# lixiaobai09/xgnn

Hardware: AMD Instinct MI355X
Metric: sampled edges/s + feature-extract GB/s per epoch-step (higher is better)
Workload: dtype u32 ids / f32 rows (bit copy)

## Files before the change

xgnn_amd/csrc/engine/engine.cc:

```cpp
#include "engine.h"
#include "team.h"
#include "../labor_hash.h"
#include "../row_formats.h"

#include <fcntl.h>
#include <pthread.h>
#include <sys/mman.h>
#include <signal.h>
#include <sys/stat.h>
#include <sys/wait.h>
#include <unistd.h>

#include <algorithm>
#include <atomic>
#include <chrono>
#include <condition_variable>
#include <cstdio>
#include <cstdlib>
#include <cstring>
#include <fstream>
#include <iostream>
#include <memory>
#include <mutex>
#include <random>
// ... 130 lines not shown
      if (kv.count("queue_timeout_s")) cfg.queue_timeout_s = std::stod(kv["queue_timeout_s"]);
      if (!(cfg.queue_timeout_s > 0))
        fatal(__FILE__, __LINE__, "arch5: queue_timeout_s = " + kv["queue_timeout_s"] + ": a positive number of seconds");
      cfg.num_worker = cfg.num_sample_worker + cfg.num_train_worker;
      break;
    }
    case kArch6:
      SAM_CHECK(kv.count("num_worker"), "arch6 needs num_worker");
      cfg.num_worker = std::stoull(kv["num_worker"]);
      SAM_CHECK(cfg.num_worker >= 1, "num_worker >= 1");
      break;
    default:
      fatal(__FILE__, __LINE__, "only arch0 (CPU), arch1 (standalone), arch3 (dedicated), arch4 (dedicated with prefetch), "
                                "arch5 (factored) and arch6 (SGNN/XGNN) are built; see DESIGN.md");
  }
  if (cfg.sample_type != GGMS_RANDOM_WALK) {
    SAM_CHECK(kv.count("num_fanout") && kv.count("fanout"), "khop sampling needs num_fanout/fanout");
    size_t nf = std::stoull(kv["num_fanout"]);
    std::stringstream ss(kv["fanout"]);
    for (size_t i = 0; i < nf; ++i) {
      size_t f = 0;
      ss >> f;
      SAM_CHECK(f > 0, "fanout: num_fanout positive integers expected");
      cfg.fanout.push_back(f);
    }
  } else {
    cfg.random_walk_length = std::stoull(kv["random_walk_length"]);
    cfg.random_walk_restart_prob = std::stod(kv["random_walk_restart_prob"]);
    cfg.num_random_walk = std::stoull(kv["num_random_walk"]);
    cfg.num_neighbor = std::stoull(kv["num_neighbor"]);
    SAM_CHECK(cfg.random_walk_length > 0 && cfg.num_random_walk > 0 && cfg.num_neighbor > 0,
              "random walk needs random_walk_length, num_random_walk and num_neighbor >= 1");
    cfg.fanout.assign(cfg.num_layer, cfg.num_neighbor);
  }
  if (kv.count("use_dist_graph")) {
    cfg.dist_graph_percentage = std::stod(kv["use_dist_graph"]);
    cfg.use_dist_graph = cfg.dist_graph_percentage > 0.0;
  }
  if (kv.count("part_cache") && kv["part_cache"] == "True") {
    SAM_CHECK(cfg.arch == kArch6, "partition cache can only be used in arch6");
    cfg.part_cache = true;
  }
  if (kv.count("gpu_extract") && kv["gpu_extract"] == "True") cfg.gpu_extract = (cfg.arch == kArch6);
  if (kv.count("replicate_percentage")) cfg.replicate_percentage = std::stod(kv["replicate_percentage"]);
  if (kv.count("presample_epoch")) cfg.presample_epoch = std::stoull(kv["presample_epoch"]);
  if (kv.count("seed")) { cfg.has_seed = true; cfg.seed = std::stoull(kv["seed"]); }
  if (kv.count("hash_table")) cfg.direct_table = kv["hash_table"] != "hashed";
  if (kv.count("lookahead")) cfg.lookahead = std::stoull(kv["lookahead"]);
  if (kv.count("staged_serial_epochs")) cfg.staged_serial_epochs = std::stoull(kv["staged_serial_epochs"]);
  if (kv.count("staged_serial_steps")) cfg.staged_serial_steps = std::stoull(kv["staged_serial_steps"]);
  if (kv.count("extract_streams")) cfg.extract_streams = std::max<size_t>(1, std::min<size_t>(2, std::stoull(kv["extract_streams"])));
  if (const char *e = getenv("SAMGRAPH_EXTRACT_STREAMS")) cfg.extract_streams = (e[0] == '1') ? 1 : 2;
  if (kv.count("pipelines")) cfg.pipelines = std::max<size_t>(1, std::min<size_t>(4, std::stoull(kv["pipelines"])));
  if (cfg.lookahead + 1 < cfg.pipelines) cfg.pipelines = cfg.lookahead + 1;
  if (cfg.arch == kArch5) {
    cfg.lookahead = 0;
    cfg.pipelines = 1;
  }
  SAM_CHECK(cfg.sample_type >= GGMS_KHOP0 && cfg.sample_type <= GGMS_KHOP_LABOR, "unknown sample type");
  if (cfg.sample_type == GGMS_KHOP_LABOR && cfg.arch == kArch0)
    fatal(__FILE__, __LINE__, "arch0: _sample_type 8 (khop_labor) is not supported: the CPU engine has no sampler for "
                              "it; it samples with khop0 or khop2");
  cfg.labor_seed = cfg.has_seed ? cfg.seed : (uint64_t)std::chrono::system_clock::now().time_since_epoch().count();
  if (kv.count("feat_out_dtype")) {
    static const std::map<std::string, int> names = {{"f32", GGMS_F32}, {"f16", GGMS_F16}, {"bf16", GGMS_BF16}};
    const std::string v = kv["feat_out_dtype"];
    if (!names.count(v))
      fatal(__FILE__, __LINE__, "feat_out_dtype = " + v + ": the converting gather delivers f32, f16 or bf16");
    cfg.feat_out_dtype = names.at(v);
    if (cfg.arch == kArch0)
      fatal(__FILE__, __LINE__, "arch0: feat_out_dtype is not built for the CPU engine: its extractor copies rows, it does "
                                "not convert them");
    if (cfg.arch == kArch6 && !cfg.gpu_extract && cfg.cache_percentage < 1.0)
      fatal(__FILE__, __LINE__, "arch6: feat_out_dtype needs gpu_extract = True or cache_percentage 1.0: the host-staged "
                                "tier's rows land in the batch by hipMemcpyAsync, which does not convert");
  }
  if (kv.count("feat_store_dtype")) {
    const std::string v = kv["feat_store_dtype"];
    const auto name = kFeatDtypeNames.find(v);
    if (name == kFeatDtypeNames.end() || !ggms::quantiser_writes(name->second))
      fatal(__FILE__, __LINE__, "feat_store_dtype = " + v + ": unknown store type; the GPU quantiser writes F16, BF16, "
                                "F8E4M3, F8E5M2 or Q8ROW");
    cfg.feat_store_dtype = name->second;
    if (cfg.arch == kArch0)
      fatal(__FILE__, __LINE__, "arch0: feat_store_dtype needs a GPU: the table is encoded by a kernel, and the CPU engine "
                                "has no GPU; quantise the dataset offline (datagen.quantize_features)");
    if (cfg.arch == kArch5 || cfg.arch == kArch6)
      fatal(__FILE__, __LINE__, std::string(cfg.arch == kArch5 ? "arch5" : "arch6") + ": feat_store_dtype is not built: the "
                                "process that loads the dataset forks its workers and must not initialise the GPU before it "
                                "forks; quantise the dataset offline (datagen.quantize_features)");
    if (cfg.feat_store_dtype == GGMS_Q8ROW && cfg.feat_out_dtype < 0) fatal(__FILE__, __LINE__, kQ8RowNeedsOutDtype);
  }
  if (kv.count("task")) {
    const std::string v = kv["task"];
    if (v != "node_classification" && v != "link_prediction")
      fatal(__FILE__, __LINE__, "task = " + v + ": node_classification (the default) or link_prediction");
    cfg.link_prediction = v == "link_prediction";
  }
  if (cfg.link_prediction) {
    static const char *const arch_names[] = {"arch0", "arch1", "arch2", "arch3", "arch4", "arch5", "arch6", "arch7"};
    if (cfg.arch != kArch1)
      fatal(__FILE__, __LINE__, std::string(arch_names[cfg.arch]) + ": task = link_prediction is not built: edge seeds, "
                                "negative sampling and the pair ids run in arch1's sampling chain only");
    if (cfg.sample_type == GGMS_RANDOM_WALK)
      fatal(__FILE__, __LINE__, "task = link_prediction with _sample_type 3 (random_walk) is not built: the pair ids are "
                                "the k-hop batch's seed ids");
// ... 599 lines not shown
  const size_t isz = num_cache_node / P + (p < num_cache_node % P ? 1 : 0) + 1;
  std::vector<uint32_t> pip(isz);
  size_t ecount = 0;
  for (uint32_t v = p; v < num_cache_node; v += P) ecount += indptr[v + 1] - indptr[v];
  std::vector<uint32_t> pix(std::max<size_t>(ecount, 1));
  uint32_t cnt = 0;
  for (uint32_t v = p; v < num_cache_node; v += P) {
    const uint32_t ne = indptr[v + 1] - indptr[v];
    pip[v / P] = cnt;
    std::memcpy(&pix[cnt], &indices[indptr[v]], ne * 4ull);
    cnt += ne;
  }
  pip[isz - 1] = cnt;
  part_indptr_.assign(P + 1, nullptr);
  part_indices_.assign(P + 1, nullptr);
  part_indptr_[p] = dev_upload(pip.data(), isz * 4, stream_);
  part_indices_[p] = dev_upload(pix.data(), ecount * 4, stream_);
  SAM_HIP(hipStreamSynchronize(stream_));
  if (P > 1) {
    SAM_HIP(hipIpcGetMemHandle(&shared_->graph_indptr[p], part_indptr_[p]));
    SAM_HIP(hipIpcGetMemHandle(&shared_->graph_indices[p], part_indices_[p]));
    shared_->indptr_words[p] = isz;
    shared_->indices_words[p] = ecount;
    Barrier("graph shards published");
    for (uint32_t q = 0; q < P; ++q) {
      if (q == p) continue;
      part_indptr_[q] = OpenPeer(shared_->graph_indptr[q], q, shared_->indptr_words[q] * 4, "graph indptr shard");
      part_indices_[q] = OpenPeer(shared_->graph_indices[q], q, shared_->indices_words[q] * 4, "graph indices shard");
    }
    Barrier("graph shards opened");
  }
  part_indptr_[P] = dev_upload(ds.indptr.ptr, ds.indptr.bytes, stream_);
  SAM_HIP(hipStreamSynchronize(stream_));
  part_indices_[P] = (void *)map_host(ds.indices.ptr, ds.indices.bytes);
  SAM_CHECK(P <= GGMS_MAX_PARTS, "use_dist_graph: at most GGMS_MAX_PARTS topology shards");
  graph_.part_indptr = (const ggms_id_t *const *)part_indptr_.data();
  graph_.part_indices = (const ggms_id_t *const *)part_indices_.data();
  graph_.num_part = P;
  graph_.num_cache_node = num_cache_node;
}

void Engine::ComputeBounds() {
  const uint32_t L = (uint32_t)cfg.fanout.size();
  max_seeds_ = (size_t)(cfg.batch_size * 1.25) + 1;
  if (cfg.link_prediction) max_seeds_ = cfg.batch_size * (2 + cfg.num_negative);
  max_input_.resize(L);
  max_edges_.resize(L);
  SAM_GGMS(ggms_sample_batch_capacity(max_seeds_, cfg.fanout.data(), L, max_input_.data(), max_edges_.data(), &max_unique_));
  if (cfg.arch == kArch4)
    SAM_GGMS(ggms_sample_batch_prefetch_capacity(max_seeds_, cfg.fanout.data(), L, (const ggms_id_t *)ds.indptr.ptr,
                                                 ds.num_node, cfg.prefetch_max_edges, &max_prefetch_edges_, &max_unique_));
}

void Engine::SampleInit(int worker_id, const std::string &ctx) {
  SAM_CHECK(data_ready_, "samgraph_data_init first");
  if (cfg.arch == kArch5) {
    SAM_CHECK(role_ == kRoleNone, "arch5: a process is one sampler or one trainer (one sample_init or one train_init)");
    SAM_CHECK(worker_id >= 0 && (size_t)worker_id < cfg.num_sample_worker, "arch5: sample_init(worker_id) with 0 <= "
              "worker_id < num_sample_worker = " + std::to_string(cfg.num_sample_worker));
    role_ = kRoleSampler;
  }
  worker_id_ = worker_id;
  device_ = parse_device(ctx);
  trainer_device_ = Dedicated() ? cfg.trainer_device : device_;
  if (trainer_device_ != device_) EnablePeerAccess();
  SAM_HIP(hipSetDevice(device_));
  SAM_HIP(hipStreamCreateWithFlags(&stream_, hipStreamNonBlocking));
  if (cfg.arch != kArch5) {
    SAM_HIP(hipSetDevice(trainer_device_));
    SAM_HIP(hipStreamCreateWithFlags(&stream_extract_, hipStreamNonBlocking));
    if (cfg.extract_streams > 1) SAM_HIP(hipStreamCreateWithFlags(&stream_extract2_, hipStreamNonBlocking));
    SAM_HIP(hipSetDevice(device_));
  }
  UploadGraph();
  ShufflerInit();
  const uint32_t L = (uint32_t)cfg.fanout.size();
  ComputeBounds();
  std::memset(&ht_, 0, sizeof(ht_));
  ht_.direct = cfg.direct_table ? 1 : 0;
  ht_.o2n_size = cfg.direct_table ? ds.num_node : ggms_hashtable_num_buckets(max_unique_);
  ht_.n2o_size = max_unique_;
  SAM_HIP(hipMalloc(&ht_.o2n, ht_.o2n_size * (cfg.direct_table ? 8 : 16)));
  SAM_HIP(hipMalloc((void **)&ht_.n2o, max_unique_ * 4));
  SAM_HIP(hipMalloc((void **)&ht_.num_items_dev, 16));
  SAM_GGMS(ggms_hashtable_init(&ht_, stream_));
  std::memset(&extra_, 0, sizeof(extra_));
  if (cfg.sample_type == GGMS_WEIGHTED_KHOP || cfg.sample_type == GGMS_WEIGHTED_KHOP_HASH_DEDUP) {
    d_prob_ = dev_upload(ds.prob_table.ptr, ds.prob_table.bytes, stream_);
    d_alias_ = dev_upload(ds.alias_table.ptr, ds.alias_table.bytes, stream_);
    extra_.prob_table = (const float *)d_prob_;
    extra_.alias_table = (const ggms_id_t *)d_alias_;
  }
  if (cfg.sample_type == GGMS_WEIGHTED_KHOP_PREFIX) {
    d_prob_ = dev_upload(ds.prob_table.ptr, ds.prob_table.bytes, stream_);
    extra_.prob_table = (const float *)d_prob_;
  }
  extra_.random_walk_length = cfg.random_walk_length;
  extra_.random_walk_restart_prob = cfg.random_walk_restart_prob;
  extra_.num_random_walk = cfg.num_random_walk;
  if (cfg.sample_type == GGMS_KHOP_LABOR) {
    num_states_ = 0;
    states_ = nullptr;
  } else {
    num_states_ = ggms_random_states_count(cfg.sample_type, cfg.fanout.data(), L, max_seeds_, cfg.num_random_walk);
    size_t max_in = 0;
    for (auto v : max_input_) max_in = std::max(max_in, v);
    num_states_ = std::max(num_states_, (max_in + 127) / 128 * 8);
    num_states_ = std::max(num_states_, (max_in + 1023) / 1024 * 256);
    if (cfg.sample_type == GGMS_RANDOM_WALK)
      num_states_ = std::max(num_states_, ggms_random_walk_num_states(max_in, cfg.num_random_walk));
    SAM_HIP(hipMalloc(&states_, num_states_ * GGMS_RNG_STATE_BYTES));
    const uint64_t seed = cfg.has_seed ? cfg.seed + 1000003ull * worker_id
                                       : (uint64_t)std::chrono::system_clock::now().time_since_epoch().count();
    SAM_GGMS(ggms_random_states_init(states_, num_states_, seed, stream_));
  }
  ws_bytes_ = cfg.arch == kArch4 ? ggms_sample_batch_prefetch_workspace_bytes(cfg.sample_type, max_seeds_, cfg.fanout.data(),
                                                                          L, &extra_, max_prefetch_edges_)
                                 : ggms_sample_batch_workspace_bytes(cfg.sample_type, max_seeds_, cfg.fanout.data(), L, &extra_);
  SAM_HIP(hipMalloc(&ws_, ws_bytes_));
  pipes_.assign(cfg.pipelines, Pipe{});
  for (size_t p = 0; p < pipes_.size(); ++p) {
    Pipe &P = pipes_[p];
    SAM_HIP(hipEventCreateWithFlags(&P.rng_done, hipEventDisableTiming));
    if (p == 0) {
      P.stream = stream_;
      P.ht = ht_;
      P.ws = ws_;
      continue;
    }
    SAM_HIP(hipStreamCreateWithFlags(&P.stream, hipStreamNonBlocking));
    P.ht = ht_;
    SAM_HIP(hipMalloc(&P.ht.o2n, ht_.o2n_size * (cfg.direct_table ? 8 : 16)));
    SAM_HIP(hipMalloc((void **)&P.ht.n2o, max_unique_ * 4));
    SAM_HIP(hipMalloc((void **)&P.ht.num_items_dev, 16));
    SAM_GGMS(ggms_hashtable_init(&P.ht, stream_));
    SAM_HIP(hipMalloc(&P.ws, ws_bytes_));
  }
  if (cfg.link_prediction && cfg.exclude_seed_edges) {
    drop_ws_bytes_ = ggms_drop_pair_edges_workspace_bytes(cfg.batch_size, max_edges_.data(), L);
    SAM_CHECK(drop_ws_bytes_ > 0, "exclude_seed_edges: the batch bounds are out of ggms_drop_pair_edges' range");
    for (Pipe &P : pipes_) SAM_HIP(hipMalloc(&P.drop_ws, drop_ws_bytes_));
  }
  if (cfg.edge_ids) {
    eid_ws_bytes_ = ggms_edge_positions_workspace_bytes(max_edges_.data(), L);
    SAM_CHECK(eid_ws_bytes_ > 0, "edge_ids: the batch bounds are out of ggms_edge_positions' range");
    for (Pipe &P : pipes_) SAM_HIP(hipMalloc(&P.eid_ws, eid_ws_bytes_));
  }
  SAM_HIP(hipStreamSynchronize(stream_));
  prof.Resize(cfg.num_epoch, num_global_step_);
  if (cfg.UsePresample()) {
    auto t0 = std::chrono::steady_clock::now();
    if (worker_id_ == 0) Presample();
    if (cfg.arch == kArch5) {
      if (worker_id_ == 0) PublishRanking();
      else WaitRankingReady();
    } else {
      Barrier("presample ranking");
    }
    prof.LogInit( 8, std::chrono::duration<double>(std::chrono::steady_clock::now() - t0).count());
  }
  if (cfg.arch == kArch5) {
    sbatch_ = std::make_unique<Batch>();
    Batch *b = sbatch_.get();
    b->sampler.Alloc(max_edges_, max_unique_, max_seeds_, cfg.sample_type == GGMS_RANDOM_WALK);
    SAM_HIP(hipEventCreateWithFlags(&b->ev_sampled, hipEventDisableTiming));
    SAM_HIP(hipEventCreateWithFlags(&b->ev_done, hipEventDisableTiming));
    QueueMap();
  }
  sample_ready_ = true;
}

void Engine::EnablePeerAccess() {
  int can = 0;
  SAM_HIP(hipDeviceCanAccessPeer(&can, trainer_device_, device_));
  if (!can)
    fatal(__FILE__, __LINE__, "arch3: GPU " + std::to_string(trainer_device_) + " (trainer_ctx) cannot access GPU " +
                                  std::to_string(device_) + " (sampler_ctx) (hipDeviceCanAccessPeer): the trainer GPU "
                                  "reads each sampled batch from the sampler GPU's memory, which needs peer access");
  SAM_HIP(hipSetDevice(trainer_device_));
  const hipError_t e = hipDeviceEnablePeerAccess(device_, 0);
  if (e == hipErrorPeerAccessAlreadyEnabled) (void)hipGetLastError();
  else SAM_HIP(e);
  SAM_HIP(hipSetDevice(device_));
  log_info("arch3: peer access GPU " + std::to_string(trainer_device_) + " -> GPU " + std::to_string(device_) + " enabled");
}

void Engine::Presample() {
  const uint32_t L = (uint32_t)cfg.fanout.size();
  const size_t n_train = ds.num_train;
  const size_t steps = (n_train + cfg.batch_size - 1) / cfg.batch_size;
  const bool closure = cfg.cache_policy == 4 ;
  std::vector<uint32_t> data((const uint32_t *)ds.train_set.ptr, (const uint32_t *)ds.train_set.ptr + n_train);
  uint32_t *d_train = nullptr, *d_freq = nullptr;
  uint64_t *d_counts = nullptr;
  SAM_HIP(hipMalloc((void **)&d_train, std::max<size_t>(n_train, 1) * 4));
  SAM_HIP(hipMalloc((void **)&d_freq, ds.num_node * 4));
  SAM_HIP(hipMalloc((void **)&d_counts, CountsBytes(L)));
  SAM_HIP(hipMemsetAsync(d_freq, 0, ds.num_node * 4, stream_));
  uint32_t *d_visit = nullptr, *d_closure = nullptr;
  void *d_cws = nullptr;
// ... 287 lines not shown
    b->trainer.Alloc(max_edges_, max_unique_, max_seeds_, cfg.sample_type == GGMS_RANDOM_WALK);
    SAM_HIP(hipMalloc(&b->feat, max_unique_ * batch_feat_row_bytes()));
    SAM_HIP(hipMalloc((void **)&b->label, max_seeds_ * 8));
    if (cfg.link_prediction) {
      SAM_HIP(hipMalloc((void **)&b->edge_ids, cfg.batch_size * 4));
      SAM_HIP(hipMalloc((void **)&b->seed_ids, max_seeds_ * 4));
      if (cfg.exclude_seed_edges) {
        SAM_HIP(hipMalloc((void **)&b->excluded_dev, L * 8));
        SAM_HIP(hipHostMalloc((void **)&b->excluded, L * 8));
        std::memset(b->excluded, 0, L * 8);
      }
    }
    if (cfg.edge_ids) {
      b->eid.assign(L, nullptr);
      b->efeat.assign(L, nullptr);
      for (uint32_t i = 0; i < L; ++i) {
        SAM_HIP(hipMalloc((void **)&b->eid[i], std::max<size_t>(max_edges_[i], 4) * 4));
        if (cfg.edge_feat) SAM_HIP(hipMalloc(&b->efeat[i], std::max<size_t>(max_edges_[i] * ds.edge_feat_row_bytes(), 16)));
      }
    }
    if (StagedHostTier()) {
      if (cache_table_) {
        for (uint32_t **p : {&b->miss_src, &b->miss_dst, &b->hit_src, &b->hit_dst}) SAM_HIP(hipMalloc((void **)p, max_unique_ * 4));
        SAM_HIP(hipMalloc(&b->idx_ws, ggms_cache_index_workspace_bytes(max_unique_)));
        SAM_HIP(hipMalloc(&b->miss_rows_dev, max_unique_ * row_bytes));
      }
      SAM_HIP(hipEventCreateWithFlags(&b->ev_ids, hipEventDisableTiming));
      SAM_HIP(hipHostMalloc(&b->miss_rows_host, max_unique_ * row_bytes));
      SAM_HIP(hipHostMalloc((void **)&b->miss_ids_host, max_unique_ * 4));
    }
    SAM_HIP(hipHostMalloc((void **)&b->counts, CountsBytes(L)));
    std::memset(b->counts, 0, CountsBytes(L));
    SAM_HIP(hipEventCreateWithFlags(&b->ev_seeds, hipEventDisableTiming));
    SAM_HIP(hipEventCreateWithFlags(&b->ev_label, hipEventDisableTiming));
    SAM_HIP(hipEventCreate(&b->ev_xstart));
    SAM_HIP(hipEventCreate(&b->ev_done));
    SAM_GGMS(ggms_launch_timer_create(&b->gather_timer));
    if (BatchSampledElsewhere()) SAM_GGMS(ggms_launch_timer_create(&b->handoff_timer));
    if (Dedicated()) {
      SAM_HIP(hipSetDevice(device_));
      b->sampler.Alloc(max_edges_, max_unique_, max_seeds_, cfg.sample_type == GGMS_RANDOM_WALK);
    } else {
      b->sampler = b->trainer;
    }
    SAM_HIP(hipEventCreate(&b->ev_start));
    SAM_HIP(hipEventCreate(&b->ev_sampled));
    if (cfg.arch == kArch4) {
      SAM_HIP(hipEventCreate(&b->ev_expand));
      SAM_HIP(hipEventCreate(&b->ev_final));
    }
    SAM_HIP(hipSetDevice(trainer_device_));
    slots_.push_back(std::move(b));
  }
  train_ready_ = true;
}

void Engine::Init() {
  if (cfg.arch == kArch0) {
    CpuInit();
    return;
  }
  DataInit();
  const std::string ctx = "cuda:" + std::to_string(cfg.sampler_device);
  SampleInit(0, ctx);
  TrainInit(0, "cuda:" + std::to_string(cfg.trainer_device));
}

void Engine::Start() {
  if (Dedicated()) ExtractStart(0);
}

void Engine::Shutdown() {
  shutdown_ = true;
  bg_stop_ = true;
  pool_cv_.notify_all();
  if (bg_.joinable()) bg_.join();
  if (cfg.arch == kArch0) CpuShutdown();
  for (auto &P : pipes_)
    if (P.stream) (void)hipStreamSynchronize(P.stream);
  if (stream_) (void)hipStreamSynchronize(stream_);
  if (stream_extract_) (void)hipStreamSynchronize(stream_extract_);
  if (stream_extract2_) (void)hipStreamSynchronize(stream_extract2_);
}

Batch *Engine::AcquireSlot(bool background) {
  for (;;) {
    {
      std::lock_guard<std::mutex> lk(pool_mu_);
      for (auto &b : slots_)
        if (!b->in_use && b->refs.load() == 0) { b->in_use = true; return b.get(); }
    }
    if (bg_stop_) return nullptr;
    if (!background) return nullptr;
    std::this_thread::sleep_for(std::chrono::microseconds(20));
  }
}

void Engine::RunSampleOnce(bool background) {
  if (IsArch5Sampler()) {
    SendOne();
    return;
  }
  if (background) {
    (void)EnqueueOne(true);
    return;
  }
  ++fg_calls_;
  while (fg_enqueued_ < fg_calls_ + cfg.lookahead && EnqueueOne(false)) ++fg_enqueued_;
}

bool Engine::EnqueueOne(bool background) {
  if (cfg.arch == kArch0) return CpuEnqueueOne(background);
  SAM_CHECK(train_ready_, "engine not initialised");
  struct RestoreDevice {
    int dev = -1;
    ~RestoreDevice() { if (dev >= 0) (void)hipSetDevice(dev); }
  } restore;
  if (Dedicated()) SAM_HIP(hipGetDevice(&restore.dev));
  SAM_HIP(hipSetDevice(device_));
  Batch *b = AcquireSlot(background);
  if (!b) return false;
  if (cfg.arch == kArch5) {
    if (!Receive(b)) {
      std::lock_guard<std::mutex> lk(pool_mu_);
      b->in_use = false;
      return false;
    }
    ++enq_count_;
    EnqueueGather(b, nullptr);
    return true;
  }
  Pipe &P = pipes_[enq_count_ % pipes_.size()];
  hipStream_t ss = P.stream;
  if (!ShufflerNext(b, ss)) {
    std::lock_guard<std::mutex> lk(pool_mu_);
    b->in_use = false;
    return false;
  }
  ++enq_count_;
  SAM_HIP(hipEventRecord(b->ev_start, ss));
  SampleInto(b, P);
  EnqueueGather(b, ss);
  return true;
}

void Engine::SampleInto(Batch *b, Pipe &P) {
  const uint32_t L = (uint32_t)cfg.fanout.size();
  const BatchArrays &s = b->sampler;
  ggms_sample_extra_t extra = extra_;
  extra.data = s.data.data();
  extra.seeds_distinct = BatchSeedsDistinct(cur_step_ * cfg.batch_size, b->num_seeds) ? 1u : 0u;
  extra.labor_salt = ggms::labor_batch_salt(cfg.labor_seed, b->key / num_global_step_, b->key % num_global_step_);
  if (cfg.link_prediction) {
    uint64_t *forced = s.counts_dev + GGMS_COUNT_LINK_FORCED(L);
    SAM_HIP(hipMemsetAsync(forced, 0, 8, P.stream));
    const uint32_t salt = ggms::fmix32(extra.labor_salt ^ 0x6c696e6bu);
    SAM_GGMS(ggms_link_seeds(&graph_, b->edge_ids, b->num_pos, cfg.num_negative, cfg.negative_mode, salt, s.output_nodes,
                             forced, P.stream));
    extra.seeds_distinct = 0;
  }
  if (pipes_.size() > 1 && cfg.sample_type != GGMS_KHOP0 && cfg.sample_type != GGMS_KHOP_LABOR) {
    extra.rng_wait = last_rng_done_;
    extra.rng_done = P.rng_done;
    last_rng_done_ = P.rng_done;
  }
  ggms_hashtable_t ht = P.ht;
  ht.n2o = s.input_nodes;
  ht.n2o_size = max_unique_;
  if (cfg.arch == kArch4)
    SAM_GGMS(ggms_sample_batch_prefetch(cfg.sample_type, &graph_, s.output_nodes, b->num_seeds, cfg.fanout.data(), L, &ht,
                                        states_, num_states_, s.row.data(), s.col.data(), s.counts_dev, &extra,
                                        max_prefetch_edges_, (ggms_event_t)b->ev_expand, (ggms_event_t)b->ev_final, P.ws,
                                        ws_bytes_, P.stream));
  else
    SAM_GGMS(ggms_sample_batch(cfg.sample_type, &graph_, s.output_nodes, b->num_seeds, cfg.fanout.data(), L, &ht, states_,
                               num_states_, s.row.data(), s.col.data(), s.counts_dev, &extra, P.ws, ws_bytes_, P.stream));
  P.ht.version = ht.version;
  if (cfg.link_prediction) {
    const ggms_id_t *ids = nullptr;
    SAM_GGMS(ggms_sample_batch_seed_ids(cfg.sample_type, b->num_seeds, cfg.fanout.data(), L, &extra, P.ws, &ids));
    SAM_HIP(hipMemcpyAsync(b->seed_ids, ids, b->num_seeds * 4, hipMemcpyDeviceToDevice, P.stream));
    if (cfg.exclude_seed_edges) {
      SAM_HIP(hipMemsetAsync(b->excluded_dev, 0, L * 8, P.stream));
      SAM_GGMS(ggms_drop_pair_edges(ids, ids + b->num_pos, b->num_pos, cfg.exclude_seed_edges, s.row.data(), s.col.data(),
                                    max_edges_.data(), L, s.counts_dev, b->excluded_dev, P.drop_ws, drop_ws_bytes_,
                                    P.stream));
      SAM_HIP(hipMemcpyAsync(b->excluded, b->excluded_dev, L * 8, hipMemcpyDeviceToHost, P.stream));
    }
  }
  if (cfg.edge_ids) {
    SAM_GGMS(ggms_edge_positions(&graph_, ds.num_edge, s.input_nodes, max_unique_, s.row.data(), s.col.data(),
                                 b->eid.data(), max_edges_.data(), L, s.counts_dev, P.eid_ws, eid_ws_bytes_, P.stream));
  }
  SAM_HIP(hipMemsetAsync(s.counts_dev + GGMS_COUNT_MISS(L), 0, 8, P.stream));
  SAM_HIP(hipEventRecord(b->ev_sampled, P.stream));
}

void Engine::EnqueueGather(Batch *b, hipStream_t ss) {
  const uint32_t L = (uint32_t)cfg.fanout.size();
  uint64_t *n_in = b->trainer.counts_dev + GGMS_COUNT_INPUT(L), *n_miss = b->trainer.counts_dev + GGMS_COUNT_MISS(L);
  const bool remote = BatchSampledElsewhere();
  if (!remote) SAM_GGMS(ggms_extract(b->label, label_src_, b->trainer.output_nodes, b->num_seeds, 1, GGMS_I64, ss));
  const bool mock = ds.feat_mask != 0xffffffffu;
  const bool can_miss = num_cached_nodes_ < ds.num_node;
  const bool gather_counts = cfg.UseGPUCache() && (mock || ((num_replica_ || cache_table_) && can_miss));
  static const bool lean_off = [] { const char *e = getenv("SAMGRAPH_LEAN_EXTRACT"); return e && e[0] == '0'; }();
  b->lean = !lean_off && !StagedHostTier() && !gather_counts && !node_access_dev_;
  if (!remote && b->lean) {
    SAM_HIP(hipMemcpyAsync(b->counts, b->trainer.counts_dev, CountsBytes(L), hipMemcpyDeviceToHost, ss));
    SAM_HIP(hipEventRecord(b->ev_done, ss));
  } else if (!remote) {
    SAM_HIP(hipEventRecord(b->ev_label, ss));
  }
  hipStream_t xs = (b->lean && stream_extract2_ && (enq_count_ & 1)) ? stream_extract2_ : stream_extract_;
  if (remote) SAM_HIP(hipSetDevice(trainer_device_));
  const bool arch4 = cfg.arch == kArch4;
  if (cfg.arch == kArch5) Unpack(b, xs);
  else SAM_HIP(hipStreamWaitEvent(xs, arch4 ? b->ev_final : b->ev_sampled, 0));
  if (remote) {
    if (cfg.arch == kArch3) Handoff(b, xs);
    if (arch4) {
      Handoff(b, xs, kHandoffIds);
      SAM_HIP(hipMemsetAsync(n_miss, 0, 8, xs));
    }
    SAM_GGMS(ggms_extract(b->label, label_src_, b->trainer.output_nodes, b->num_seeds, 1, GGMS_I64, xs));
  }
  if (cfg.edge_feat)
    for (uint32_t i = 0; i < L; ++i)
      SAM_GGMS(ggms_gather_scatter(b->efeat[i], d_edge_feat_, b->eid[i], nullptr, max_edges_[i],
                                   b->trainer.counts_dev + GGMS_COUNT_EDGES(i), ds.edge_feat_dim, ds.edge_feat_dtype, xs));
  if (b->lean) SAM_GGMS(ggms_launch_timer_arm(b->gather_timer));
  else SAM_HIP(hipEventRecord(b->ev_xstart, xs));
  const int out_dtype = batch_feat_dtype();
  uint32_t dyn_seq = 0;
  if (cfg.dynamic_cache) {
    if (++dyn_seq_ == 0) {
      SAM_GGMS(ggms_dynamic_cache_reset(dyn_stamps_, ds.num_node, xs));
      dyn_seq_ = 1;
    }
    dyn_seq = dyn_seq_;
  }
  if (StagedHostTier()) {
    StagedExtract(b, ss, xs);
  } else if (cfg.dynamic_cache) {
    SAM_GGMS(ggms_extract_dynamic(b->feat, b->trainer.input_nodes, max_unique_, n_in, dyn_stamps_, dyn_seq,
                                  dyn_prev_ ? dyn_prev_->feat : nullptr, feat_src_, ds.feat_dim, ds.feat_dtype, n_miss, xs));
  } else if (cfg.UseGPUCache() && (mock || num_replica_)) {
    if (gather_counts) SAM_HIP(hipMemsetAsync(n_miss, 0, GGMS_NUM_TIERS * 8, xs));
    ggms_feature_tiers_t tiers{};
    tiers.table = cache_table_;
    tiers.replica = d_replica_;
    tiers.num_replica = num_replica_;
    tiers.parts = (const void *const *)cache_parts_.data();
    tiers.num_part = std::max<uint32_t>(1, num_cache_part_);
    tiers.my_part = cfg.part_cache ? (uint32_t)worker_id_ : 0;
    tiers.host_feat = feat_src_;
    tiers.host_row_mask = mock ? ds.feat_mask : 0;
    SAM_GGMS(ggms_extract_tiered_convert(b->feat, b->trainer.input_nodes, max_unique_, n_in, &tiers, ds.feat_dim,
                                         ds.feat_dtype, out_dtype, gather_counts ? n_miss : nullptr, xs));
  } else if (cfg.UseGPUCache()) {
    SAM_GGMS(ggms_extract_cached_convert(b->feat, b->trainer.input_nodes, max_unique_, n_in, cache_table_,
                                         (const void *const *)cache_parts_.data(), num_cache_part_, feat_src_, ds.feat_dim,
                                         ds.feat_dtype, out_dtype, (cache_table_ && can_miss) ? n_miss : nullptr, xs));
  } else {
    SAM_GGMS(ggms_gather_scatter_convert(b->feat, feat_src_, b->trainer.input_nodes, nullptr, max_unique_, n_in,
                                         ds.feat_dim, ds.feat_dtype, out_dtype, ds.feat_mask, xs));
  }
// ... 297 lines not shown
```

xgnn_amd/csrc/engine/engine.h:

```cpp
#pragma once

#include <hip/hip_runtime.h>

#include <atomic>
#include <condition_variable>
#include <cstdint>
#include <deque>
#include <map>
#include <memory>
#include <mutex>
#include <string>
#include <thread>
#include <unordered_map>
#include <vector>

#include "../../../include/ggms.h"
#include "../../../include/samgraph.h"

namespace sam {

[[noreturn]] void fatal(const char *file, int line, const std::string &msg);
#define SAM_CHECK(cond, msg)                                   \
  do {                                                         \
    if (!(cond)) ::sam::fatal(__FILE__, __LINE__, std::string("Check failed: " #cond " ") + (msg)); \
  } while (0)
#define SAM_HIP(call)                                          \
  do {                                                         \
    hipError_t e_ = (call);                                    \
    if (e_ != hipSuccess) ::sam::fatal(__FILE__, __LINE__, std::string(#call " -> ") + hipGetErrorString(e_)); \
  } while (0)
#define SAM_GGMS(call)                                         \
  do {                                                         \
    int rc_ = (call);                                          \
    if (rc_ != 0) ::sam::fatal(__FILE__, __LINE__, std::string(#call " -> ") + ggms_last_error()); \
  } while (0)
void log_info(const std::string &msg);
int parse_device(const std::string &ctx);

enum Arch { kArch0 = 0, kArch1, kArch2, kArch3, kArch4, kArch5, kArch6, kArch7 };
struct RunConfig {
  std::unordered_map<std::string, std::string> raw;
  std::string dataset_path;
  int arch = kArch1;
  int sample_type = GGMS_KHOP3;
  size_t batch_size = 8000, num_epoch = 1;
  int cache_policy = 0;
  double cache_percentage = 0.0;
  size_t num_layer = 0;
  std::vector<size_t> fanout;
  size_t random_walk_length = 0, num_random_walk = 0, num_neighbor = 0;
  double random_walk_restart_prob = 0.0;
  size_t num_worker = 1;
  size_t num_sample_worker = 0, num_train_worker = 0, queue_depth = 0;
  double queue_timeout_s = 300.0;
  int sampler_device = 0, trainer_device = 0;
  bool trainer_on_host = false;
  size_t omp_thread_num = 1;
  bool use_dist_graph = false;
  double dist_graph_percentage = 0.0;
  bool part_cache = false, gpu_extract = false;
  double replicate_percentage = 0.0;
  bool configured = false;
  bool has_seed = false;
  uint64_t seed = 0;
  uint64_t labor_seed = 0;
  bool direct_table = true;
  size_t lookahead = 2;
  size_t extract_streams = 2;
  size_t pipelines = 1;
  size_t presample_epoch = 0;
  bool dynamic_cache = false;
  size_t prefetch_max_edges = (size_t)1 << 26;
  int feat_out_dtype = -1;
  int feat_store_dtype = -1;
  bool link_prediction = false;
  uint32_t num_negative = 1;
  int negative_mode = GGMS_NEG_EXCLUDE;
  uint32_t exclude_seed_edges = 0;
  int feat_learnable = -1;
  float feat_lr = 0.0f, feat_eps = 1e-10f;
  bool edge_ids = false, edge_feat = false;
  size_t staged_serial_epochs = 0;
  size_t staged_serial_steps = 0;
  bool UsePresample() const {
    return UseGPUCache() && (cache_policy == 2  || cache_policy == 4 );
  }
  bool UseGPUCache() const { return cache_percentage > 0 && arch != kArch1; }
};

struct HostArray {
  void *ptr = nullptr;
  size_t bytes = 0;
  bool mapped_file = false, shared_anon = false, owned = false;
};
struct Dataset {
  size_t num_node = 0, num_edge = 0, num_class = 0, feat_dim = 0;
  int feat_dtype = GGMS_F32;
  size_t num_train = 0, num_valid = 0, num_test = 0;
  HostArray indptr, indices, feat, label, train_set, valid_set, test_set, ranking_nodes, prob_table, alias_table;
  HostArray train_edge_set;
  std::vector<uint32_t> all_edges;
  const uint32_t *train_edges = nullptr;
  size_t num_train_edge = 0;
  bool feat_is_fake = false;
  bool feat_is_zero = false;
  uint32_t feat_mask = 0xffffffffu;
  size_t feat_rows = 0;
  size_t feat_row_bytes() const { return ggms_row_bytes(feat_dtype, feat_dim); }
  size_t edge_feat_dim = 0;
  int edge_feat_dtype = GGMS_F32;
  HostArray edge_feat;
  size_t edge_feat_row_bytes() const { return edge_feat_dim * ggms_dtype_bytes(edge_feat_dtype); }
};

class Profiler {
 public:
  void Resize(size_t num_epoch, size_t num_step);
  void LogInit(int item, double v) { init_[item] = v; }
  void LogInitAdd(int item, double v) { init_[item] += v; }
  void LogStep(uint64_t key, int item, double v);
  void LogStepAdd(uint64_t key, int item, double v);
  void LogEpochAdd(uint64_t key, int item, double v);
// ... 141 lines not shown
  void Handoff(Batch *b, hipStream_t xs, HandoffPart part = kHandoffAll);
  void EnqueueGather(Batch *b, hipStream_t ss);

  enum Role { kRoleNone, kRoleSampler, kRoleTrainer };
  Role role_ = kRoleNone;
  struct QueueCtl;
  QueueCtl *queue_ = nullptr;
  char *queue_slots_ = nullptr;
  char *queue_slots_dev_ = nullptr;
  size_t queue_depth_ = 0;
  ggms_queue_layout_t qlay_{};
  std::unique_ptr<Batch> sbatch_;
  void ComputeBounds();
  void QueueInit();
  void QueueMap();
  ggms_queue_header_t *QueueHeader(uint64_t pos) const;
  bool QueueWait(const uint64_t *word, uint64_t want, const char *what, bool stoppable);
  void PublishRanking();
  void WaitRankingReady();
  void Arch5TrainerInit(int worker_id, const std::string &ctx);
  void SendOne();
  bool Receive(Batch *b);
  void Unpack(Batch *b, hipStream_t xs);

  bool data_ready_ = false, sample_ready_ = false, train_ready_ = false, shutdown_ = false;
  int worker_id_ = 0, device_ = 0;
  int trainer_device_ = 0;
  hipStream_t stream_ = nullptr;
  hipStream_t stream_extract_ = nullptr;
  hipStream_t stream_extract2_ = nullptr;
  uint32_t *d_indptr_ = nullptr, *d_indices_ = nullptr;
  std::vector<void *> part_indptr_, part_indices_;
  ggms_graph_t graph_{};
  ggms_hashtable_t ht_{};
  ggms_sample_extra_t extra_{};
  void *d_prob_ = nullptr, *d_alias_ = nullptr;
  void *states_ = nullptr;
  size_t num_states_ = 0;
  void *ws_ = nullptr;
  size_t ws_bytes_ = 0;
  struct Pipe {
    hipStream_t stream = nullptr;
    ggms_hashtable_t ht{};
    void *ws = nullptr;
    hipEvent_t rng_done = nullptr;
    void *drop_ws = nullptr;
    void *eid_ws = nullptr;
  };
  size_t drop_ws_bytes_ = 0;
  size_t eid_ws_bytes_ = 0;
  void *d_edge_feat_ = nullptr;
  uint64_t link_excluded_ = 0;
  std::vector<Pipe> pipes_;
  size_t enq_count_ = 0;
  hipEvent_t last_rng_done_ = nullptr;
  void SampleInto(Batch *b, Pipe &P);
  size_t max_seeds_ = 0, max_unique_ = 0;
  size_t max_prefetch_edges_ = 0;
  uint64_t *dyn_stamps_ = nullptr;
  uint32_t dyn_seq_ = 0;
  Batch *dyn_prev_ = nullptr;
  std::vector<size_t> max_input_, max_edges_;
  std::vector<uint32_t> shuf_host_;
  uint32_t *shuf_dev_ = nullptr;
  size_t num_data_ = 0, num_local_data_ = 0, num_local_step_ = 0, num_global_step_ = 0;
  size_t global_step_offset_ = 0, global_data_offset_ = 0;
  size_t cur_epoch_ = 0, cur_step_ = 0;
  bool shuf_initialized_ = false;
  bool train_distinct_ = false;
  std::vector<std::pair<size_t, size_t>> pad_pairs_;
  bool BatchSeedsDistinct(size_t offset, size_t size) const;
  uint32_t *cache_table_ = nullptr;
  std::vector<void *> cache_parts_;
  uint32_t num_cache_part_ = 0;
  size_t num_cached_nodes_ = 0;
  size_t num_replica_ = 0;
  void *d_replica_ = nullptr;
  void *d_feat_ = nullptr;
  void *d_feat_state_ = nullptr;
  hipEvent_t ev_grad_ = nullptr, ev_updated_ = nullptr;
  const void *feat_src_ = nullptr;
  const void *label_src_ = nullptr;
  std::vector<std::unique_ptr<Batch>> slots_;
  std::deque<Batch *> pool_;
  std::mutex pool_mu_;
  std::condition_variable pool_cv_;
  Batch *current_ = nullptr;
  std::thread bg_;
  size_t fg_calls_ = 0, fg_enqueued_ = 0;
  std::atomic<bool> bg_stop_{false};
  std::atomic<bool> bg_running_{false};
  struct Shared;
  Shared *shared_ = nullptr;
};

}
```

Baseline: 5.312 billion.

## Auto-select sampling pipeline and extract stream counts by online trial

Adds a runtime trial that times several (pipelines, extract streams) candidates over the first batches with events, then keeps the fastest and frees unused pipelines. Pipe setup is split into InitPipe and FreePipe so pipelines can be added and removed after init, and the active pipeline and stream counts are now separate from the allocated ones. The goal is to choose the overlap setting that suits the workload instead of using fixed defaults. The cost is stream drains and candidate switching during the trial steps, plus extra memory for pipelines while the trial runs.

```diff
diff --git a/xgnn_amd/csrc/engine/engine.cc b/xgnn_amd/csrc/engine/engine.cc
--- a/xgnn_amd/csrc/engine/engine.cc
+++ b/xgnn_amd/csrc/engine/engine.cc
@@ -206,6 +206,7 @@
   if (kv.count("extract_streams")) cfg.extract_streams = std::max<size_t>(1, std::min<size_t>(2, std::stoull(kv["extract_streams"])));
   if (const char *e = getenv("SAMGRAPH_EXTRACT_STREAMS")) cfg.extract_streams = (e[0] == '1') ? 1 : 2;
   if (kv.count("pipelines")) cfg.pipelines = std::max<size_t>(1, std::min<size_t>(4, std::stoull(kv["pipelines"])));
+  if (kv.count("streams_trial")) cfg.streams_trial = kv["streams_trial"] != "0" && kv["streams_trial"] != "False";
   if (cfg.lookahead + 1 < cfg.pipelines) cfg.pipelines = cfg.lookahead + 1;
   if (cfg.arch == kArch5) {
     cfg.lookahead = 0;
@@ -911,6 +912,36 @@
                                                  ds.num_node, cfg.prefetch_max_edges, &max_prefetch_edges_, &max_unique_));
 }
 
+void Engine::InitPipe(size_t p) {
+  Pipe &P = pipes_[p];
+  SAM_HIP(hipEventCreateWithFlags(&P.rng_done, hipEventDisableTiming));
+  P.ht = ht_;
+  if (p == 0) {
+    P.stream = stream_;
+    P.ws = ws_;
+  } else {
+    if (streams_shared_) P.stream = stream_extract2_;
+    else SAM_HIP(hipStreamCreateWithFlags(&P.stream, hipStreamNonBlocking));
+    SAM_HIP(hipMalloc(&P.ht.o2n, ht_.o2n_size * (cfg.direct_table ? 8 : 16)));
+    SAM_HIP(hipMalloc((void **)&P.ht.n2o, max_unique_ * 4));
+    SAM_HIP(hipMalloc((void **)&P.ht.num_items_dev, 16));
+    SAM_GGMS(ggms_hashtable_init(&P.ht, stream_));
+    SAM_HIP(hipMalloc(&P.ws, ws_bytes_));
+  }
+  if (drop_ws_bytes_) SAM_HIP(hipMalloc(&P.drop_ws, drop_ws_bytes_));
+  if (eid_ws_bytes_) SAM_HIP(hipMalloc(&P.eid_ws, eid_ws_bytes_));
+}
+
+void Engine::FreePipe(size_t p) {
+  SAM_CHECK(p > 0 && p < pipes_.size(), "FreePipe: pipeline 0 stays");
+  Pipe &P = pipes_[p];
+  for (void *q : {(void *)P.ht.o2n, (void *)P.ht.n2o, (void *)P.ht.num_items_dev, P.ws, P.drop_ws, P.eid_ws})
+    if (q) SAM_HIP(hipFree(q));
+  if (P.stream && P.stream != stream_extract2_) SAM_HIP(hipStreamDestroy(P.stream));
+  SAM_HIP(hipEventDestroy(P.rng_done));
+  P = Pipe{};
+}
+
 void Engine::SampleInit(int worker_id, const std::string &ctx) {
   SAM_CHECK(data_ready_, "samgraph_data_init first");
   if (cfg.arch == kArch5) {
@@ -977,34 +1008,16 @@
                                                                           L, &extra_, max_prefetch_edges_)
                                  : ggms_sample_batch_workspace_bytes(cfg.sample_type, max_seeds_, cfg.fanout.data(), L, &extra_);
   SAM_HIP(hipMalloc(&ws_, ws_bytes_));
-  pipes_.assign(cfg.pipelines, Pipe{});
-  for (size_t p = 0; p < pipes_.size(); ++p) {
-    Pipe &P = pipes_[p];
-    SAM_HIP(hipEventCreateWithFlags(&P.rng_done, hipEventDisableTiming));
-    if (p == 0) {
-      P.stream = stream_;
-      P.ht = ht_;
-      P.ws = ws_;
-      continue;
-    }
-    SAM_HIP(hipStreamCreateWithFlags(&P.stream, hipStreamNonBlocking));
-    P.ht = ht_;
-    SAM_HIP(hipMalloc(&P.ht.o2n, ht_.o2n_size * (cfg.direct_table ? 8 : 16)));
-    SAM_HIP(hipMalloc((void **)&P.ht.n2o, max_unique_ * 4));
-    SAM_HIP(hipMalloc((void **)&P.ht.num_items_dev, 16));
-    SAM_GGMS(ggms_hashtable_init(&P.ht, stream_));
-    SAM_HIP(hipMalloc(&P.ws, ws_bytes_));
-  }
   if (cfg.link_prediction && cfg.exclude_seed_edges) {
     drop_ws_bytes_ = ggms_drop_pair_edges_workspace_bytes(cfg.batch_size, max_edges_.data(), L);
     SAM_CHECK(drop_ws_bytes_ > 0, "exclude_seed_edges: the batch bounds are out of ggms_drop_pair_edges' range");
-    for (Pipe &P : pipes_) SAM_HIP(hipMalloc(&P.drop_ws, drop_ws_bytes_));
   }
   if (cfg.edge_ids) {
     eid_ws_bytes_ = ggms_edge_positions_workspace_bytes(max_edges_.data(), L);
     SAM_CHECK(eid_ws_bytes_ > 0, "edge_ids: the batch bounds are out of ggms_edge_positions' range");
-    for (Pipe &P : pipes_) SAM_HIP(hipMalloc(&P.eid_ws, eid_ws_bytes_));
-  }
+  }
+  pipes_.assign(cfg.pipelines, Pipe{});
+  for (size_t p = 0; p < pipes_.size(); ++p) InitPipe(p);
   SAM_HIP(hipStreamSynchronize(stream_));
   prof.Resize(cfg.num_epoch, num_global_step_);
   if (cfg.UsePresample()) {
@@ -1398,6 +1411,7 @@
     SAM_HIP(hipSetDevice(trainer_device_));
     slots_.push_back(std::move(b));
   }
+  PlanStreams();
   train_ready_ = true;
 }
 
@@ -1476,7 +1490,8 @@
     EnqueueGather(b, nullptr);
     return true;
   }
-  Pipe &P = pipes_[enq_count_ % pipes_.size()];
+  if (trial_.active) TrialBeforeEnqueue();
+  Pipe &P = pipes_[enq_count_ % act_pipes_];
   hipStream_t ss = P.stream;
   if (!ShufflerNext(b, ss)) {
     std::lock_guard<std::mutex> lk(pool_mu_);
@@ -1487,7 +1502,145 @@
   SAM_HIP(hipEventRecord(b->ev_start, ss));
   SampleInto(b, P);
   EnqueueGather(b, ss);
+  if (trial_.active) TrialAfterEnqueue();
   return true;
+}
+
+bool Engine::GatherCounts() const {
+  const bool mock = ds.feat_mask != 0xffffffffu;
+  const bool can_miss = num_cached_nodes_ < ds.num_node;
+  return cfg.UseGPUCache() && (mock || ((num_replica_ || cache_table_) && can_miss));
+}
+
+bool Engine::LeanBatches() const {
+  static const bool lean_off = [] { const char *e = getenv("SAMGRAPH_LEAN_EXTRACT"); return e && e[0] == '0'; }();
+  return !lean_off && !StagedHostTier() && !GatherCounts() && !node_access_dev_;
+}
+
+static std::string streams_name(const StreamsChoice &c) {
+  return "(" + std::to_string(c.pipelines) + ", " + std::to_string(c.extract_streams) + ")";
+}
+
+void Engine::LogStreams(const char *how) {
+  static const std::map<std::string, int> codes = {{"trial", 1}, {"explicit", 2}, {"forced", 3}, {"too few batches", 4}};
+  std::string msg = "streams: ";
+  if (!trial_.cands.empty()) {
+    msg += "candidates (pipelines, extract streams)";
+    for (size_t i = 0; i < trial_.cands.size(); ++i) {
+      char ms[32] = "not timed";
+      if (i < trial_.ms.size() && trial_.ms[i] > 0) std::snprintf(ms, sizeof ms, "%.4f ms/step", trial_.ms[i]);
+      msg += std::string(i ? ", " : " ") + streams_name(trial_.cands[i]) + " " + ms;
+      if (i < trial_.ms.size() && 45 + i < (size_t)Profiler::kMaxInit) prof.LogInit(45 + (int)i, trial_.ms[i]);
+    }
+    msg += "; ";
+  }
+  msg += "using " + std::to_string(act_pipes_) + " sampling pipeline(s), " + std::to_string(act_xs_) +
+         " extract stream(s) [" + how + "]";
+  prof.LogInit(42, (double)act_pipes_);
+  prof.LogInit(43, (double)act_xs_);
+  prof.LogInit(44, (double)codes.at(how));
+  std::fprintf(stderr, "[samgraph-amd] %s\n", msg.c_str());
+}
+
+void Engine::PlanStreams() {
+  act_pipes_ = std::max<size_t>(1, pipes_.size());
+  act_xs_ = stream_extract2_ ? 2 : 1;
+  if (cfg.arch == kArch0 || IsArch5Sampler()) return;
+  const bool is_explicit = cfg.raw.count("pipelines") || cfg.raw.count("extract_streams") ||
+                           getenv("SAMGRAPH_EXTRACT_STREAMS") || !cfg.streams_trial;
+  const bool lean = LeanBatches();
+  if (!lean) act_xs_ = 1;
+  if (is_explicit) return LogStreams("explicit");
+  StreamsRules rules;
+  rules.lookahead = cfg.lookahead;
+  rules.one_pipeline = cfg.arch == kArch5;
+  rules.dynamic_cache = cfg.dynamic_cache;
+  rules.feat_learnable = cfg.feat_learnable >= 0;
+  rules.lean = lean;
+  std::vector<StreamsChoice> cands = streams_filter(streams_candidates(cfg.sample_type == GGMS_KHOP0), rules);
+  if (BatchSampledElsewhere() || !lean || cands.size() < 2) return LogStreams("forced");
+  trial_.cands = cands;
+  trial_.block = streams_trial_block(num_local_step_, cands.size());
+  if (trial_.block == 0) return LogStreams("too few batches");
+  size_t max_pipes = 1, max_xs = 1;
+  bool both = false;
+  for (const StreamsChoice &c : cands) {
+    max_pipes = std::max(max_pipes, c.pipelines);
+    max_xs = std::max(max_xs, c.extract_streams);
+    both = both || (c.pipelines > 1 && c.extract_streams > 1);
+  }
+  SAM_HIP(hipSetDevice(device_));
+  if (max_xs > 1 && !stream_extract2_) SAM_HIP(hipStreamCreateWithFlags(&stream_extract2_, hipStreamNonBlocking));
+  streams_shared_ = stream_extract2_ && !both;
+  const size_t have = pipes_.size();
+  if (max_pipes > have) pipes_.resize(max_pipes);
+  for (size_t p = have; p < pipes_.size(); ++p) InitPipe(p);
+  SAM_HIP(hipStreamSynchronize(stream_));
+  SAM_HIP(hipEventCreate(&trial_.ev_begin));
+  for (hipEvent_t &e : trial_.ev_end) SAM_HIP(hipEventCreate(&e));
+  trial_.ms.assign(cands.size(), 0.0);
+  trial_.cand = trial_.n = 0;
+  trial_.active = true;
+  UseStreams(cands[0]);
+}
+
+void Engine::DrainStreams() {
+  for (Pipe &P : pipes_)
+    if (P.stream) SAM_HIP(hipStreamSynchronize(P.stream));
+  SAM_HIP(hipStreamSynchronize(stream_extract_));
+  if (stream_extract2_) SAM_HIP(hipStreamSynchronize(stream_extract2_));
+}
+
+void Engine::UseStreams(const StreamsChoice &c) {
+  SAM_CHECK(c.pipelines >= 1 && c.pipelines <= pipes_.size() && c.extract_streams >= 1 &&
+                (c.extract_streams == 1 || stream_extract2_) && !(streams_shared_ && c.pipelines > 1 && c.extract_streams > 1),
+            "streams trial: candidate " + streams_name(c) + " was not allocated");
+  act_pipes_ = c.pipelines;
+  act_xs_ = c.extract_streams;
+  last_rng_done_ = nullptr;
+}
+
+void Engine::TrialBeforeEnqueue() {
+  StreamsTrial &T = trial_;
+  if (T.n == 0) {
+    DrainStreams();
+    UseStreams(T.cands[T.cand]);
+    T.best_ms = 0;
+  }
+  if (T.n == kTrialWarmup) DrainStreams();
+  if (T.n == kTrialWarmup || T.n == kTrialWarmup + T.block)
+    SAM_HIP(hipEventRecord(T.ev_begin, pipes_[enq_count_ % act_pipes_].stream));
+}
+
+void Engine::TrialAfterEnqueue() {
+  StreamsTrial &T = trial_;
+  ++T.n;
+  if (T.n != kTrialWarmup + T.block && T.n != kTrialWarmup + kTrialBlocks * T.block) return;
+  SAM_HIP(hipEventRecord(T.ev_end[0], stream_extract_));
+  if (act_xs_ > 1) SAM_HIP(hipEventRecord(T.ev_end[1], stream_extract2_));
+  DrainStreams();
+  float ms = 0, ms2 = 0;
+  SAM_HIP(hipEventElapsedTime(&ms, T.ev_begin, T.ev_end[0]));
+  if (act_xs_ > 1) SAM_HIP(hipEventElapsedTime(&ms2, T.ev_begin, T.ev_end[1]));
+  ms = std::max(ms, ms2);
+  if (T.best_ms == 0 || ms < T.best_ms) T.best_ms = ms;
+  if (T.n < kTrialWarmup + kTrialBlocks * T.block) return;
+  T.ms[T.cand] = T.best_ms / (double)T.block;
+  T.n = 0;
+  if (++T.cand == T.cands.size()) EndTrial(choose_streams(T.ms.data(), T.ms.size()));
+}
+
+void Engine::EndTrial(size_t chosen) {
+  StreamsTrial &T = trial_;
+  T.active = false;
+  UseStreams(T.cands[chosen]);
+  while (pipes_.size() > act_pipes_) {
+    FreePipe(pipes_.size() - 1);
+    pipes_.pop_back();
+  }
+  SAM_HIP(hipEventDestroy(T.ev_begin));
+  for (hipEvent_t e : T.ev_end) SAM_HIP(hipEventDestroy(e));
+  LogStreams("trial");
 }
 
 void Engine::SampleInto(Batch *b, Pipe &P) {
@@ -1505,7 +1658,7 @@
                              forced, P.stream));
     extra.seeds_distinct = 0;
   }
-  if (pipes_.size() > 1 && cfg.sample_type != GGMS_KHOP0 && cfg.sample_type != GGMS_KHOP_LABOR) {
+  if (act_pipes_ > 1 && cfg.sample_type != GGMS_KHOP0 && cfg.sample_type != GGMS_KHOP_LABOR) {
     extra.rng_wait = last_rng_done_;
     extra.rng_done = P.rng_done;
     last_rng_done_ = P.rng_done;
@@ -1549,16 +1702,15 @@
   if (!remote) SAM_GGMS(ggms_extract(b->label, label_src_, b->trainer.output_nodes, b->num_seeds, 1, GGMS_I64, ss));
   const bool mock = ds.feat_mask != 0xffffffffu;
   const bool can_miss = num_cached_nodes_ < ds.num_node;
-  const bool gather_counts = cfg.UseGPUCache() && (mock || ((num_replica_ || cache_table_) && can_miss));
-  static const bool lean_off = [] { const char *e = getenv("SAMGRAPH_LEAN_EXTRACT"); return e && e[0] == '0'; }();
-  b->lean = !lean_off && !StagedHostTier() && !gather_counts && !node_access_dev_;
+  const bool gather_counts = GatherCounts();
+  b->lean = LeanBatches();
   if (!remote && b->lean) {
     SAM_HIP(hipMemcpyAsync(b->counts, b->trainer.counts_dev, CountsBytes(L), hipMemcpyDeviceToHost, ss));
     SAM_HIP(hipEventRecord(b->ev_done, ss));
   } else if (!remote) {
     SAM_HIP(hipEventRecord(b->ev_label, ss));
   }
-  hipStream_t xs = (b->lean && stream_extract2_ && (enq_count_ & 1)) ? stream_extract2_ : stream_extract_;
+  hipStream_t xs = (b->lean && act_xs_ > 1 && (enq_count_ & 1)) ? stream_extract2_ : stream_extract_;
   if (remote) SAM_HIP(hipSetDevice(trainer_device_));
   const bool arch4 = cfg.arch == kArch4;
   if (cfg.arch == kArch5) Unpack(b, xs);
diff --git a/xgnn_amd/csrc/engine/engine.h b/xgnn_amd/csrc/engine/engine.h
--- a/xgnn_amd/csrc/engine/engine.h
+++ b/xgnn_amd/csrc/engine/engine.h
@@ -16,6 +16,7 @@
 
 #include "../../../include/ggms.h"
 #include "../../../include/samgraph.h"
+#include "streams_trial.h"
 
 namespace sam {
 
@@ -68,6 +69,7 @@
   size_t lookahead = 2;
   size_t extract_streams = 2;
   size_t pipelines = 1;
+  bool streams_trial = true;
   size_t presample_epoch = 0;
   bool dynamic_cache = false;
   size_t prefetch_max_edges = (size_t)1 << 26;
@@ -315,7 +317,29 @@
   void *d_edge_feat_ = nullptr;
   uint64_t link_excluded_ = 0;
   std::vector<Pipe> pipes_;
+  void InitPipe(size_t p);
+  void FreePipe(size_t p);
   size_t enq_count_ = 0;
+  size_t act_pipes_ = 1, act_xs_ = 1;
+  struct StreamsTrial {
+    bool active = false;
+    std::vector<StreamsChoice> cands;
+    std::vector<double> ms;
+    size_t cand = 0, n = 0;
+    size_t block = 0;
+    double best_ms = 0;
+    hipEvent_t ev_begin = nullptr, ev_end[2] = {nullptr, nullptr};
+  } trial_;
+  bool streams_shared_ = false;
+  bool GatherCounts() const;
+  bool LeanBatches() const;
+  void PlanStreams();
+  void UseStreams(const StreamsChoice &c);
+  void DrainStreams();
+  void TrialBeforeEnqueue();
+  void TrialAfterEnqueue();
+  void EndTrial(size_t chosen);
+  void LogStreams(const char *how);
   hipEvent_t last_rng_done_ = nullptr;
   void SampleInto(Batch *b, Pipe &P);
   size_t max_seeds_ = 0, max_unique_ = 0;
diff --git a/xgnn_amd/csrc/engine/streams_trial.h b/xgnn_amd/csrc/engine/streams_trial.h
--- /dev/null
+++ b/xgnn_amd/csrc/engine/streams_trial.h
@@ -0,0 +1,64 @@
+#pragma once
+
+#include <cstddef>
+#include <vector>
+
+namespace sam {
+
+struct StreamsChoice {
+  size_t pipelines = 1, extract_streams = 1;
+  bool operator==(const StreamsChoice &o) const { return pipelines == o.pipelines && extract_streams == o.extract_streams; }
+};
+
+struct StreamsRules {
+  size_t lookahead = 2;
+  bool one_pipeline = false;
+  bool dynamic_cache = false;
+  bool feat_learnable = false;
+  bool lean = true;
+};
+
+constexpr size_t kTrialWarmup = 3;
+constexpr size_t kTrialBlocks = 2;
+constexpr size_t kTrialBlock = 12;
+constexpr size_t kTrialMinBlock = 4;
+constexpr double kTrialMargin = 0.02;
+
+inline std::vector<StreamsChoice> streams_candidates(bool khop0) {
+  if (khop0) return {{2, 2}, {2, 1}};
+  return {{1, 1}, {1, 2}, {2, 1}};
+}
+
+inline bool streams_legal(const StreamsChoice &c, const StreamsRules &r) {
+  if (c.pipelines < 1 || c.extract_streams < 1) return false;
+  if (c.pipelines > r.lookahead + 1) return false;
+  if (r.one_pipeline && c.pipelines > 1) return false;
+  if ((r.dynamic_cache || r.feat_learnable || !r.lean) && c.extract_streams > 1) return false;
+  return true;
+}
+
+inline std::vector<StreamsChoice> streams_filter(const std::vector<StreamsChoice> &cands, const StreamsRules &r) {
+  std::vector<StreamsChoice> out;
+  for (const StreamsChoice &c : cands)
+    if (streams_legal(c, r)) out.push_back(c);
+  return out;
+}
+
+inline size_t streams_trial_block(size_t steps, size_t num_cand) {
+  if (num_cand == 0) return 0;
+  const size_t each = steps / num_cand;
+  if (each < kTrialWarmup + kTrialBlocks * kTrialMinBlock) return 0;
+  const size_t block = (each - kTrialWarmup) / kTrialBlocks;
+  return block < kTrialBlock ? block : kTrialBlock;
+}
+
+inline size_t choose_streams(const double *ms, size_t n, double margin = kTrialMargin) {
+  if (n == 0) return 0;
+  size_t best = 0;
+  for (size_t i = 1; i < n; ++i)
+    if (ms[i] > 0 && (!(ms[best] > 0) || ms[i] < ms[best])) best = i;
+  if (!(ms[0] > 0)) return best;
+  return ms[best] < (1.0 - margin) * ms[0] ? best : 0;
+}
+
+}
```

Result: no change. 5.296 billion (-0.3%).
